# lixilinx/psgd_tf

Measured on AMD Instinct MI355X. Metric: uvd_update_apply_params_per_sec, higher is better.
Workload: dtype f32

## Files before the change

### psgd_tf_amd/csrc/psgd_kron.hip

```cpp
#include <hip/hip_runtime.h>
#include <stdint.h>
#include <stdlib.h>
#include <algorithm>
#include <map>
#include <mutex>
#include <utility>
#include "psgd_hip.h"
#include "kron_shared.h"
#include "nanmax.h"
using psgd::amaxf;
using psgd::nmaxf;

namespace psgdk {

typedef float f32x4 __attribute__((ext_vector_type(4)));

constexpr int kThreads = 256;

enum { EPI_STORE = 0, EPI_TRIU_MAX = 1, EPI_D_MINUS = 2 };

struct GemmArgs {
  const float* A; long a_rs, a_cs;
  const float* B; long b_rs, b_cs;
  const float* A2; long a2_rs, a2_cs;
// ... 1626 lines not shown
    SmallSrc sa, sb;
    small_src_init(sa, ta, m0, hi);
    small_src_init(sb, tb, n0, hi);
    float ra[D][8], rb[D][8];
#pragma unroll
    for (int d = 0; d < D; ++d) {
      small_fetch(sa, lo + d * GK, d < n, ra[d]);
      small_fetch(sb, lo + d * GK, d < n, rb[d]);
    }
    for (int t0 = 0; t0 < n; t0 += D) {
#pragma unroll
      for (int d = 0; d < D; ++d) {
        const int t = t0 + d, buf = d & 1;
        if (t < n) {
          small_commit(sa, lo + t * GK, mul, ra[d], LA + buf * kBuf);
          small_commit(sb, lo + t * GK, 1.0f, rb[d], LB + buf * kBuf);
        }
        small_fetch(sa, lo + (t + D) * GK, t + D < n, ra[d]);
        small_fetch(sb, lo + (t + D) * GK, t + D < n, rb[d]);
        if (t < n) {
          __syncthreads();
#pragma unroll
          for (int kk = 0; kk < GK / 4; ++kk) {
            const int kr = kk * 4 + (lane >> 4);
            const float a = L.A[buf][kr][wm * 16 + (lane & 15)];
            const float b = L.B[buf][kr][wn * 16 + (lane & 15)];
            acc[0][0] = __builtin_amdgcn_mfma_f32_16x16x4f32(a, b, acc[0][0], 0, 0, 0);
          }
        }
      }
    }
    __syncthreads();
  };
  if (nk[0] > 0) run_pair(TileSrc{g.A, g.a_rs, g.a_cs, g.M}, TileSrc{g.B, g.b_cs, g.b_rs, g.N}, klo[0], khi[0], nk[0], a_mul);
  if (nk[1] > 0) run_pair(TileSrc{g.A2, g.a2_rs, g.a2_cs, g.M}, TileSrc{g.B2, g.b2_cs, g.b2_rs, g.N}, klo[1], khi[1], nk[1], -a_mul);
  gemm_epilogue<32>(g, acc, m0, n0);
}

__global__ __launch_bounds__(kThreads) void k_gemm_small(GemmBatch b) {
  __shared__ __attribute__((aligned(16))) GemmLds<32, kSmallK> L;
  int p = 0;
  while (p + 1 < b.count && (int)blockIdx.x >= b.tile_end[p]) ++p;
  const int t = blockIdx.x - (p ? b.tile_end[p - 1] : 0);
  const GemmArgs& g = b.g[p];
  const int tn = (g.N + 31) / 32;
  gemm_body_small(g, (t / tn) * 32, (t % tn) * 32, L);
}

__global__ __launch_bounds__(kThreads) void k_gemm_small_one(GemmArgs g) {
  __shared__ __attribute__((aligned(16))) GemmLds<32, kSmallK> L;
  gemm_body_small(g, blockIdx.y * 32, blockIdx.x * 32, L);
}

constexpr int kMaxGrams = 16;
struct GramBatch {
  int count;
  int tile_end[kMaxGrams];
  const float* Q[kMaxGrams];
  float* P[kMaxGrams];
  int n[kMaxGrams];
};

__host__ __device__ inline GemmArgs gram_args(const float* Q, float* P, int n) {
  GemmArgs g = {};
  g.A = Q; g.a_rs = 1; g.a_cs = n;
  g.B = Q; g.b_rs = n; g.b_cs = 1;
  g.C = P; g.ldc = n; g.M = n; g.N = n; g.K = n;
  g.epi = EPI_STORE;
  g.kmode = KHI_M | KHI_N;
  g.sym = 1;
  return g;
}

template <int T>
__global__ __launch_bounds__(kThreads) void k_gram_batched(GramBatch b) {
  int p = 0;
  while (p + 1 < b.count && (int)blockIdx.x >= b.tile_end[p]) ++p;
  const int t = blockIdx.x - (p ? b.tile_end[p - 1] : 0);
  const GemmArgs g = gram_args(b.Q[p], b.P[p], b.n[p]);
  const int tn = (g.N + T - 1) / T;
  if constexpr (T == 32) {
    __shared__ __attribute__((aligned(16))) GemmLds<32, kSmallK> L;
    gemm_body_small(g, (t / tn) * 32, (t % tn) * 32, L);
  } else {
    __shared__ __attribute__((aligned(16))) GemmLds<T, kSmallK> L;
    gemm_body<T, kSmallK>(g, (t / tn) * T, (t % tn) * T, L);
  }
}

struct TrsmArgs {
  const float* Q; int n, ldq;
  const float* X; float* Y;
  int nvec; long si, sj;
  long xi, xj;
};

__device__ __forceinline__ void trsm_body(const float* __restrict__ Q, int n, int ldq, const float* X, float* Y,
                                          int nvec, long si, long sj, long xi, long xj, int v0,
                                          float (*red)[64][33], float (*Qd)[32]) {
  if (xi == 0 && xj == 0) { xi = si; xj = sj; }
  const int lane = threadIdx.x & 63, w = threadIdx.x >> 6;
  for (int j0 = 0; j0 < n; j0 += 32) {
    const int jw = (n - j0 < 32) ? (n - j0) : 32;
    f32x4 acc[4][2];
#pragma unroll
    for (int i = 0; i < 4; ++i)
// ... 434 lines not shown
  __shared__ float Ybuf[2][512];
  trsm_reg_full_body(t, Dinv, blockIdx.x * 16, Ybuf);
}

__global__ __launch_bounds__(kThreads) void k_tri_inv512(const float* __restrict__ Q, int n, const float* __restrict__ dinv,
                                                         float* __restrict__ Inv, float* amax) {
  __shared__ float Ybuf[2][512];
  const int d = blockIdx.x >> 5, v0 = (blockIdx.x & 31) * 16;
  const long o = (long)(512 * d) * n + 512 * d;
  TrsmArgs t = {Q + o, 512, n, nullptr, Inv + o, 512, (long)n, 1L, 0L, 0L};
  trsm_reg_full_body<true>(t, dinv + (long)(16 * d) * 1024, v0, Ybuf, amax);
}

__global__ __launch_bounds__(kThreads) void k_trsm_ut_reg(TrsmArgs t, const float* __restrict__ Dinv) {
  __shared__ float Ybuf[2][512];
  trsm_reg_body(t, Dinv, blockIdx.x * 16, Ybuf);
}

struct TrsmBatch {
  int count;
  int blk_end[kMaxBatch];
  TrsmArgs t[kMaxBatch];
  const float* dinv[kMaxBatch];
};

__global__ __launch_bounds__(kThreads) void k_trsm_ut_inv_batched(TrsmBatch b, int pitch_max) {
  extern __shared__ __attribute__((aligned(16))) float dyn_lds[];
  int p = 0;
  while (p + 1 < b.count && (int)blockIdx.x >= b.blk_end[p]) ++p;
  const int blk = blockIdx.x - (p ? b.blk_end[p - 1] : 0);
  const TrsmArgs& t = b.t[p];
  const int pitch = ((t.n + 31) & ~31) + 2;
  trsm_inv_body<16>(t, b.dinv[p], blk * 16, dyn_lds, pitch, reinterpret_cast<float (*)[33]>(dyn_lds + 16 * pitch_max));
}

__global__ __launch_bounds__(kThreads) void k_trsm_ut_reg_batched(TrsmBatch b) {
  __shared__ float Ybuf[2][512];
  int p = 0;
  while (p + 1 < b.count && (int)blockIdx.x >= b.blk_end[p]) ++p;
  const int blk = blockIdx.x - (p ? b.blk_end[p - 1] : 0);
  trsm_reg_body(b.t[p], b.dinv[p], blk * 16, Ybuf);
}


struct MixBatch {
  int count, strips;
  int blk_end[kMaxLayers];
  int tile_end[kMaxLayers];
  TrsmArgs t[kMaxLayers];
  const float* dinv[kMaxLayers];
  GemmArgs g[kMaxLayers];
};

__global__ __launch_bounds__(kThreads) void k_small_stage_mixed(MixBatch b) {
  __shared__ __attribute__((aligned(16))) GemmLds<32, kSmallK> L;
  __shared__ float Ybuf[2][512];
  if ((int)blockIdx.x < b.strips) {
    int p = 0;
    while (p + 1 < b.count && (int)blockIdx.x >= b.blk_end[p]) ++p;
    const int blk = blockIdx.x - (p ? b.blk_end[p - 1] : 0);
    trsm_reg_body(b.t[p], b.dinv[p], blk * 16, Ybuf);
    return;
  }
  const int id = blockIdx.x - b.strips;
  int p = 0;
  while (p + 1 < b.count && id >= b.tile_end[p]) ++p;
  const int t = id - (p ? b.tile_end[p - 1] : 0);
  const GemmArgs& g = b.g[p];
  const int tn = (g.N + 31) / 32;
  gemm_body_small(g, (t / tn) * 32, (t % tn) * 32, L);
}

struct BalanceBatch {
  int count;
  const float* Ql[kMaxBatch]; const float* Qr[kMaxBatch];
  float* QlS[kMaxBatch]; float* QrS[kMaxBatch];
  float* dinv[kMaxBatch];
  float* scal[kMaxBatch];
  int M[kMaxBatch], N[kMaxBatch];
};

__device__ __forceinline__ float balance_rho(const float* __restrict__ Ql, const float* __restrict__ Qr, int M, int N,
                                             float (*red)[4]) {
  float ml = -INFINITY, mr = -INFINITY;
  for (int i0 = threadIdx.x; i0 < M; i0 += 8 * kThreads) {
    float x[8];
#pragma unroll
    for (int u = 0; u < 8; ++u) { const long i = min(i0 + u * kThreads, M - 1); x[u] = Ql[i * M + i]; }
#pragma unroll
    for (int u = 0; u < 8; ++u) ml = nmaxf(ml, x[u]);
  }
  for (int i0 = threadIdx.x; i0 < N; i0 += 8 * kThreads) {
    float x[8];
#pragma unroll
    for (int u = 0; u < 8; ++u) { const long i = min(i0 + u * kThreads, N - 1); x[u] = Qr[i * N + i]; }
#pragma unroll
    for (int u = 0; u < 8; ++u) mr = nmaxf(mr, x[u]);
  }
#pragma unroll
  for (int off = 32; off > 0; off >>= 1) {
    ml = nmaxf(ml, __shfl_down(ml, off, 64));
    mr = nmaxf(mr, __shfl_down(mr, off, 64));
  }
  const int lane = threadIdx.x & 63, w = threadIdx.x >> 6;
  if (lane == 0) { red[0][w] = ml; red[1][w] = mr; }
  __syncthreads();
  ml = nmaxf(nmaxf(red[0][0], red[0][1]), nmaxf(red[0][2], red[0][3]));
  mr = nmaxf(nmaxf(red[1][0], red[1][1]), nmaxf(red[1][2], red[1][3]));
  return sqrtf(ml / mr);
}

__device__ __forceinline__ void balance_body(const float* __restrict__ Ql, const float* __restrict__ Qr, int M, int N,
                                             float* QlS, float* QrS, float (*red)[4], int bid, int nblocks,
                                             float* part_l = nullptr, float* part_r = nullptr) {
  const float rho = balance_rho(Ql, Qr, M, N, red);
  const long nl = (long)M * M, nr = (long)N * N;
  const long tid = (long)bid * kThreads + threadIdx.x, nth = (long)nblocks * kThreads;
  float ml = 0.0f, mr = 0.0f;
  const bool v4 = ((reinterpret_cast<uintptr_t>(Ql) | reinterpret_cast<uintptr_t>(Qr) | reinterpret_cast<uintptr_t>(QlS) |
                    reinterpret_cast<uintptr_t>(QrS)) & 15) == 0;
  long dl = 0, dr = 0;
  if (v4) {
    const long nl4 = nl >> 2, nr4 = nr >> 2;
// ... 548 lines not shown
  return (lo >= kInvMinSmall && hi >= kInvMinN) || (lo >= 512 && hi >= 2560) || (lo >= 256 && hi >= 4096);
}

static KronWs kron_layout(char* base, int M, int N) {
  KronWs k;
  const int64_t mm = (int64_t)M * M * 4, nn = (int64_t)N * N * 4, mn = (int64_t)M * N * 4;
  int64_t off = 0;
  auto take = [&](int64_t bytes) { float* p = reinterpret_cast<float*>(base + off); off = align256(off + bytes); return p; };
  k.scal = take(256);
  k.QlS = take(mm); k.QrS = take(nn);
  k.T = take(mn); k.A = take(mn); k.X1 = take(mn); k.Bt = take(mn);
  k.g1 = take(mm); k.g2 = take(nn);
  k.dinv = take((int64_t)((M + 31) / 32 + (N + 31) / 32) * 1024 * 4);
  k.Pl = take(mm); k.Pr = take(nn);
  k.PP = k.F1 = k.F2 = k.Y0 = k.Y1 = k.Y2 = nullptr;
  k.Lr = k.Lc = k.Rr = k.Rc = k.G1 = k.G2 = k.U0 = k.U1 = k.U2 = k.U3 = nullptr;
  k.split_scratch = nullptr; k.split_cnt = nullptr; k.S0 = nullptr;
  k.sk_scratch = nullptr; k.sk_cnt = nullptr; k.pmeta = nullptr; k.pm_part = nullptr; k.te = nullptr;
  k.IcL = k.IcR = k.TpL = k.TpR = k.DXp = k.X1p = nullptr; k.TfL = k.TfR = nullptr;
  if (kron_planes(M, N)) {
    const int64_t Mp = pad128(M), Np = pad128(N), small = Mp < Np ? Mp : Np, big = Mp < Np ? Np : Mp;
    auto planes = [&](int64_t elems) { return reinterpret_cast<__bf16*>(take(elems * 6)); };
    k.PP = planes(small * small); k.F1 = planes(big * big); k.F2 = planes(big * big);
    k.Y0 = planes(Mp * Np); k.Y1 = planes(Mp * Np); k.Y2 = planes(Mp * Np);
    k.Lr = planes(Mp * Mp); k.Lc = planes(Mp * Mp); k.G1 = planes(Mp * Mp);
    k.Rr = planes(Np * Np); k.Rc = planes(Np * Np); k.G2 = planes(Np * Np);
    k.U0 = planes(Mp * Np); k.U1 = planes(Mp * Np); k.U2 = planes(Mp * Np); k.U3 = planes(Mp * Np);
    {
      const int64_t T1 = small / 128, nsp = T1 * (T1 + 1) / 2 < kGradSplitMax ? T1 * (T1 + 1) / 2 : kGradSplitMax;
      k.split_scratch = take(nsp * kGradChunks * 64 * kThreads * 4);
      k.split_cnt = reinterpret_cast<unsigned*>(take(2 * kGradSplitMax * 4));
    }
    k.S0 = planes(big * 2048);
    k.pmeta = reinterpret_cast<PlaneMeta*>(take(1024));
    k.pm_part = take(4 * 2048 * 4);
    k.te = reinterpret_cast<int*>(take((int64_t)kTeSlots * kTeLd * kTeLd * 4));
    if (kron_inv_route(M, N)) {
      k.IcL = planes(Mp * Mp); k.TpL = planes(Mp * Mp); k.TfL = take(mm);
      k.IcR = planes(Np * Np); k.TpR = planes(Np * Np); k.TfR = take(nn);
      k.DXp = planes(Mp * Np); k.X1p = planes(Mp * Np);
    }
    if (kron_t128(M, N) <= kSkMaxTiles) {
      k.sk_scratch = take((int64_t)kSkItems * 64 * kThreads * 4);
      k.sk_cnt = reinterpret_cast<unsigned*>(take(kSkMaxTiles * 4));
    }
  }
  k.total = off;
  return k;
}

static int g_gemm_x3 = 1;
static int g_force_gemm = 0;
static int g_small_deep = 1;

static int x3_host_mode(const float* P, long rs, long cs) {
  if (rs == 1 && cs > 0 && cs < (1L << 23)) return X3_XROW;
  if (cs == 1 && rs > 0 && rs < (1L << 22) && (rs & 3) == 0 && (reinterpret_cast<uintptr_t>(P) & 15) == 0) return X3_KVEC;
  return X3_EDGE;
}
static void x3_host_modes(const GemmArgs& g, int& ma, int& mb) {
  ma = x3_host_mode(g.A, g.a_rs, g.a_cs);
  mb = x3_host_mode(g.B, g.b_cs, g.b_rs);
  if (g.A2 && (x3_host_mode(g.A2, g.a2_rs, g.a2_cs) != ma || x3_host_mode(g.B2, g.b2_cs, g.b2_rs) != mb)) ma = X3_EDGE;
  if (ma == X3_EDGE || mb == X3_EDGE) ma = mb = X3_EDGE;
}

template <bool LITE>
static void launch_x3(const GemmArgs& g, dim3 grid, hipStream_t st) {
  int ma, mb;
  x3_host_modes(g, ma, mb);
  if (ma == X3_KVEC && mb == X3_XROW) hipLaunchKernelGGL((k_gemm_x3<X3_KVEC, X3_XROW, LITE>), grid, dim3(kThreads), 0, st, g);
  else if (ma == X3_KVEC && mb == X3_KVEC) hipLaunchKernelGGL((k_gemm_x3<X3_KVEC, X3_KVEC, LITE>), grid, dim3(kThreads), 0, st, g);
  else if (ma == X3_XROW && mb == X3_XROW) hipLaunchKernelGGL((k_gemm_x3<X3_XROW, X3_XROW, LITE>), grid, dim3(kThreads), 0, st, g);
  else if (ma == X3_XROW && mb == X3_KVEC) hipLaunchKernelGGL((k_gemm_x3<X3_XROW, X3_KVEC, LITE>), grid, dim3(kThreads), 0, st, g);
  else hipLaunchKernelGGL((k_gemm_x3<X3_EDGE, X3_EDGE, LITE>), grid, dim3(kThreads), 0, st, g);
}

static int launch_gemm(const GemmArgs& g, hipStream_t st) {
  if (g.C == g.A || g.C == g.B || (g.A2 && (g.C == g.A2 || g.C == g.B2))) return PSGD_ERR_BAD_ARG;
  const long t128 = (long)((g.N + 127) / 128) * ((g.M + 127) / 128);
  const long t64 = (long)((g.N + 63) / 64) * ((g.M + 63) / 64);
  int T = t128 >= 64 ? 128 : (t64 >= 48 ? 64 : 32);
  if (g_force_gemm == 1) T = 64;
  if (g_force_gemm == 2) T = 128;
  if (g_force_gemm == 3) T = 32;
  dim3 grid((g.N + T - 1) / T, (g.M + T - 1) / T);
  if (T == 128 && g_gemm_x3 && g.lite) launch_x3<true>(g, grid, st);
  else if (T == 128 && g_gemm_x3) launch_x3<false>(g, grid, st);
  else if (T == 128) hipLaunchKernelGGL((k_gemm_f32<128, kBigK>), grid, dim3(kThreads), 0, st, g);
  else if (T == 64) hipLaunchKernelGGL((k_gemm_f32<64, kSmallK>), grid, dim3(kThreads), 0, st, g);
  else if (g_small_deep && g.K > 2 * kSmallK)
    hipLaunchKernelGGL(k_gemm_small_one, grid, dim3(kThreads), 0, st, g);
  else hipLaunchKernelGGL((k_gemm_f32<32, kSmallK>), grid, dim3(kThreads), 0, st, g);
  return (int)hipGetLastError();
}

static bool gemm_uses_x3(const GemmArgs& g) {
  const long t128 = (long)((g.N + 127) / 128) * ((g.M + 127) / 128);
  return g_gemm_x3 && (g_force_gemm == 0 ? t128 >= 64 : g_force_gemm == 2);
}

static int launch_gemm_two(const GemmArgs& a, const GemmArgs& b, hipStream_t st) {
  if (!gemm_uses_x3(a) || !gemm_uses_x3(b)) {
    const int rc = launch_gemm(a, st);
    return rc ? rc : launch_gemm(b, st);
  }
  GemmPair p;
  p.g[0] = a; p.g[1] = b;
  p.tx0 = (a.N + 127) / 128; p.tx1 = (b.N + 127) / 128;
  p.tiles0 = p.tx0 * ((a.M + 127) / 128);
  const int tiles1 = p.tx1 * ((b.M + 127) / 128);
  p.tiles1 = tiles1;
  int ma0, mb0, ma1, mb1;
  x3_host_modes(a, ma0, mb0);
  x3_host_modes(b, ma1, mb1);
  const dim3 grid(p.tiles0 + tiles1);
  if (ma0 == X3_KVEC && mb0 == X3_KVEC && ma1 == X3_XROW && mb1 == X3_XROW)
    hipLaunchKernelGGL((k_gemm_x3_pair<X3_KVEC, X3_KVEC, X3_XROW, X3_XROW>), grid, dim3(kThreads), 0, st, p);
  else if (ma0 == X3_KVEC && mb0 == X3_XROW && ma1 == X3_KVEC && mb1 == X3_XROW)
    hipLaunchKernelGGL((k_gemm_x3_pair<X3_KVEC, X3_XROW, X3_KVEC, X3_XROW>), grid, dim3(kThreads), 0, st, p);
  else {
    const int rc = launch_gemm(a, st);
    return rc ? rc : launch_gemm(b, st);
  }
  return (int)hipGetLastError();
}

static GemmArgs gemm_args(const float* A, int lda, bool ta, const float* B, int ldb, bool tb, float* C, int ldc, int M,
                          int N, int K, int kmode = 0) {
  GemmArgs g = {};
  g.A = A; g.a_rs = ta ? 1 : lda; g.a_cs = ta ? lda : 1;
  g.B = B; g.b_rs = tb ? 1 : ldb; g.b_cs = tb ? ldb : 1;
  g.C = C; g.ldc = ldc; g.M = M; g.N = N; g.K = K;
  g.epi = EPI_STORE;
  g.kmode = kmode;
  return g;
}

constexpr int kSmallKron = 512;
static inline bool kron_small(int M, int N) { return M <= kSmallKron && N <= kSmallKron; }

static void plan_apply(const float* Ql, const float* Qr, const float* G, float* out, int M, int N, const KronWs& k,
                       GemmArgs (&pre)[2], int& np, GemmArgs (&app)[3], int& na) {
// ... 318 lines not shown
        (long)((cw + 127) / 128) * ((nvec + 127) / 128) >= g_trsm_planes_min_tiles && (!Qc->meta || strip_slots > 0)) {
      P3Buf Yg = {blk, pad128(nvec), kw};
      int e;
      if (Qc->meta) {
        Yg.meta = strip_meta++; --strip_slots;
        if ((e = launch_absmax_view(Y + (long)k0 * sj, si, sj, nvec, kw, Yg, part, st))) return e;
      }
      if ((e = launch_split3(Y + (long)k0 * sj, si, sj, nvec, kw, Yg, st))) return e;
      P3Args g = p3_args(Yg, *Qc, nvec, cw, kw, 0);
      g.B.p = Qc->p + (long)(k0 / 32) * (Qc->rows * 32) + (long)c0 * 32;
      float* Yr = Y + (long)c0 * sj;
      g.e.C = Yr; g.e.ldc = si; g.e.c_cs = sj;
      g.e.D = (lazy && k0 == 0 ? X : Y) + (long)c0 * sj; g.e.ldd = si;
      g.e.epi = EPI_D_MINUS;
      return launch_p3(g, st);
    }
    GemmArgs g = {};
    g.A = Y + (long)k0 * sj; g.a_rs = si; g.a_cs = sj;
    g.B = Q + (long)k0 * n + c0; g.b_rs = n; g.b_cs = 1;
    float* Yr = Y + (long)c0 * sj;
    g.C = Yr; g.ldc = si; g.c_cs = sj;
    g.D = (lazy && k0 == 0 ? X : Y) + (long)c0 * sj; g.ldd = si;
    g.M = nvec; g.N = cw; g.K = kw;
    g.epi = EPI_D_MINUS;
    g.lite = lite;
    return launch_gemm(g, st);
  };
  const int group = kTrsmBlock * (g_trsm_group > 0 ? g_trsm_group : (n >= 8 * kTrsmBlock ? 4 : 1));
  for (int g0 = 0; g0 < n; g0 += group) {
    const int gend = (n - g0 < group) ? n : g0 + group;
    for (int j0 = g0; j0 < gend; j0 += kTrsmBlock) {
      const int jw = (gend - j0 < kTrsmBlock) ? (gend - j0) : kTrsmBlock;
      float* Yb = Y + (long)j0 * sj;
      TrsmArgs t = {Q + (long)j0 * n + j0, jw, n, (lazy && j0 == 0) ? X : Yb, Yb, nvec, si, sj, 0L, 0L};
      int e = launch_strip(t, dinv + (long)(j0 / 32) * 1024, st);
      if (e) return e;
      if (j0 + jw < gend && (e = update(j0, jw, j0 + jw, gend - j0 - jw))) return e;
    }
    if (gend < n) {
      const int e = update(g0, gend - g0, gend, n - gend);
      if (e) return e;
    }
  }
  return 0;
}

static int launch_gemm_batch(const GemmArgs* g, int count, hipStream_t st) {
  GemmBatch b;
  b.count = count;
  long t64 = 0;
  for (int p = 0; p < count; ++p) t64 += (long)((g[p].N + 63) / 64) * ((g[p].M + 63) / 64);
  const int T = t64 >= 96 ? 64 : 32;
  int tiles = 0;
  for (int p = 0; p < count; ++p) {
    b.g[p] = g[p];
    tiles += ((g[p].N + T - 1) / T) * ((g[p].M + T - 1) / T);
    b.tile_end[p] = tiles;
  }
  if (T == 64) hipLaunchKernelGGL((k_gemm_f32_batched<64>), dim3(tiles), dim3(kThreads), 0, st, b);
  else if (g_small_deep) hipLaunchKernelGGL(k_gemm_small, dim3(tiles), dim3(kThreads), 0, st, b);
  else hipLaunchKernelGGL((k_gemm_f32_batched<32>), dim3(tiles), dim3(kThreads), 0, st, b);
  return (int)hipGetLastError();
}

static int launch_gram_batch(const GemmArgs* g, int count, hipStream_t st) {
  for (int p0 = 0; p0 < count; p0 += kMaxGrams) {
    GramBatch b;
    b.count = (count - p0 < kMaxGrams) ? count - p0 : kMaxGrams;
    long t64 = 0;
    for (int p = 0; p < b.count; ++p) t64 += (long)((g[p0 + p].N + 63) / 64) * ((g[p0 + p].M + 63) / 64);
    const int T = t64 >= 96 ? 64 : 32;
    int tiles = 0;
    for (int p = 0; p < b.count; ++p) {
      const GemmArgs& a = g[p0 + p];
      b.Q[p] = a.A; b.P[p] = a.C; b.n[p] = a.M;
      tiles += ((a.N + T - 1) / T) * ((a.M + T - 1) / T);
      b.tile_end[p] = tiles;
    }
    if (T == 64) hipLaunchKernelGGL((k_gram_batched<64>), dim3(tiles), dim3(kThreads), 0, st, b);
    else hipLaunchKernelGGL((k_gram_batched<32>), dim3(tiles), dim3(kThreads), 0, st, b);
    if (hipGetLastError() != hipSuccess) return 1;
  }
  return 0;
}

static int launch_p3_two(const P3Args& a, const P3Args& b, hipStream_t st) {
  P3Pair p;
  p.g[0] = a; p.g[1] = b;
  p.tx0 = (a.e.N + 127) / 128; p.tx1 = (b.e.N + 127) / 128;
  p.tiles0 = p.tx0 * ((a.e.M + 127) / 128);
  const int tiles1 = p.tx1 * ((b.e.M + 127) / 128);
  p.tiles1 = tiles1;
  const dim3 grid(p.tiles0 + tiles1);
  const bool none = p3_no_early((p.tiles0 + tiles1) / 2 >= p3_block_slots() * 3 / 4);
  if (!a.fmt) hipLaunchKernelGGL((k_gemm_p3_pair<0, 2>), grid, dim3(kThreads), 0, st, p);
  else if (p3_uses_te(a) || p3_uses_te(b)) {
    if (none) hipLaunchKernelGGL((k_gemm_p3_pair<1, 0, true>), grid, dim3(kThreads), 0, st, p);
    else hipLaunchKernelGGL((k_gemm_p3_pair<1, 2, true>), grid, dim3(kThreads), 0, st, p);
  } else if (none) hipLaunchKernelGGL((k_gemm_p3_pair<1, 0>), grid, dim3(kThreads), 0, st, p);
  else hipLaunchKernelGGL((k_gemm_p3_pair<1, 2>), grid, dim3(kThreads), 0, st, p);
  return (int)hipGetLastError();
}

static int g_grad_rect = 1;
static int g_grad_split = 1;
constexpr int g_grad_order = 1;
static int grad_rect_chunks(int m_long, int k_long, int k_short) {
  if (!g_grad_split || !g_grad_rect || k_long == k_short) return 0;
  const int Tl = (m_long + 127) / 128, nl = Tl * (Tl + 1) / 2;
  const int ratio = (k_long + k_short / 2) / k_short;
  if (ratio < 2 || nl > kGradSplitMax) return 0;
  const int nchunk = ratio >= 7 ? 8 : ratio >= 5 ? 6 : ratio >= 3 ? 4 : 2;
// ... 715 lines not shown
  if (!f || !f->bg || hipStreamWaitEvent(f->bg, f->fork, 0) != hipSuccess) return 1;
  f->bg_live = 1;
  return 0;
}

int kron_join(KronFork* f, hipStream_t main) {
  if (f->bg_live) {
    f->bg_live = 0;
    if (hipEventRecord(f->bg_done, f->bg) != hipSuccess || hipStreamWaitEvent(main, f->bg_done, 0) != hipSuccess) return 1;
  }
  if (hipEventRecord(f->join, f->side) != hipSuccess) return 1;
  return hipStreamWaitEvent(main, f->join, 0) != hipSuccess;
}

}

using namespace psgdk;

#define KRON_LAUNCH(expr)                     \
  do {                                        \
    if ((expr) != 0) return PSGD_ERR_LAUNCH;  \
  } while (0)

static int kron_ws_check(void* ws, int64_t ws_bytes, int64_t need) {
  if (!ws || (reinterpret_cast<uintptr_t>(ws) & 255) || ws_bytes < need) return PSGD_ERR_WORKSPACE;
  return PSGD_OK;
}

extern "C" {

int psgd_kron_set_tuning(int key, int value) {
  if (key == 0) { g_force_gemm = value; return PSGD_OK; }
  if (key == 1) { g_gemm_x3 = value; return PSGD_OK; }
  if (key == 2) { g_trsm_lds = value; return PSGD_OK; }
  if (key == 3) { g_small_deep = value; return PSGD_OK; }
  if (key == 4) { g_planes = value; return PSGD_OK; }
  if (key == 6) { g_grad_split = value; return PSGD_OK; }
  if (key == 7) { g_stage_mix = value; return PSGD_OK; }
  if (key == 9) { g_overlap = value; return PSGD_OK; }
  if (key == 11) { g_trsm_inv = value; return PSGD_OK; }
  if (key == 12) { g_planes_f16 = value; return PSGD_OK; }
  if (key == 16) { g_planes_exact = value; return PSGD_OK; }
  if (key == 23) { g_inv_strip512 = value; return PSGD_OK; }
  if (key == 24) { g_inv_blk = value; return PSGD_OK; }
  if (key == 25) { g_inv_order = value; return PSGD_OK; }
  if (key == 27) { g_pair_order = value; return PSGD_OK; }
  if (key == 28) { g_tile_scales = value; return PSGD_OK; }
  if (key == 29) { g_x0_side = value; return PSGD_OK; }
  if (key == 30) { g_bg_front = value; return PSGD_OK; }
  if (key == 31) { g_fused_prologue = value; return PSGD_OK; }
  if (key == 32) { g_bg_planes = value; return PSGD_OK; }
  if (key == 33) { g_grad_rect = value; return PSGD_OK; }
  if (key == 34) { g_solve_split = value; return PSGD_OK; }
  return PSGD_ERR_BAD_ARG;
}

int64_t psgd_kron_dd_workspace_bytes(int M, int N) {
  if (M <= 0 || N <= 0) return PSGD_ERR_BAD_ARG;
  return kron_layout(nullptr, M, N).total;
}

static inline bool kron_apply_planes(int M, int N) { return kron_planes_apply(M, N) && g_planes && g_gemm_x3; }

int psgd_kron_dd_prepare_f32(const float* Ql, const float* Qr, int M, int N, void* ws, int64_t ws_bytes, void* stream) {
  if (!Ql || !Qr) return PSGD_ERR_BAD_ARG;
  if (M <= 0 || N <= 0) return PSGD_ERR_SHAPE;
  if (kron_ws_check(ws, ws_bytes, kron_layout(nullptr, M, N).total)) return PSGD_ERR_WORKSPACE;
  hipStream_t st = static_cast<hipStream_t>(stream);
  KronWs k = kron_layout(static_cast<char*>(ws), M, N);
  if (kron_apply_planes(M, N)) {
    KRON_LAUNCH(planes_prepare(Ql, Qr, M, N, k, st));
    return PSGD_OK;
  }
  GemmArgs pre[2], app[3];
  int np = 0, na = 0;
  plan_apply(Ql, Qr, Ql , k.T , M, N, k, pre, np, app, na);
  if (np == 2) KRON_LAUNCH(launch_gram_batch(pre, 2, st));
  else KRON_LAUNCH(launch_gemm(pre[0], st));
  return PSGD_OK;
}

int psgd_kron_dd_apply_prepared_f32(const float* Ql, const float* Qr, const float* G, float* out, int M, int N, void* ws,
                                    int64_t ws_bytes, void* stream) {
  if (!Ql || !Qr || !G || !out) return PSGD_ERR_BAD_ARG;
  if (M <= 0 || N <= 0) return PSGD_ERR_SHAPE;
  if (kron_ws_check(ws, ws_bytes, kron_layout(nullptr, M, N).total)) return PSGD_ERR_WORKSPACE;
  hipStream_t st = static_cast<hipStream_t>(stream);
  KronWs k = kron_layout(static_cast<char*>(ws), M, N);
  if (kron_apply_planes(M, N)) {
    KRON_LAUNCH(planes_apply(G, out, M, N, k, st));
    return PSGD_OK;
  }
  GemmArgs pre[2], app[3];
  int np = 0, na = 0;
  plan_apply(Ql, Qr, G, out, M, N, k, pre, np, app, na);
  for (int i = 0; i < na; ++i) KRON_LAUNCH(launch_gemm(app[i], st));
  return PSGD_OK;
}

int psgd_kron_dd_apply_f32(const float* Ql, const float* Qr, const float* G, float* out, int M, int N, void* ws,
                           int64_t ws_bytes, void* stream) {
  const int rc = psgd_kron_dd_prepare_f32(Ql, Qr, M, N, ws, ws_bytes, stream);
  if (rc) return rc;
  return psgd_kron_dd_apply_prepared_f32(Ql, Qr, G, out, M, N, ws, ws_bytes, stream);
}

// ... 246 lines not shown
                                    const float* const* dG, float* const* QlOut, float* const* QrOut, const int* M,
                                    const int* N, int count, float step, float tiny, void* ws, int64_t ws_bytes,
                                    void* stream) {
  if (!Ql || !Qr || !dX || !dG || !QlOut || !QrOut || !M || !N || count <= 0) return PSGD_ERR_BAD_ARG;
  const int64_t need = psgd_kron_dd_workspace_bytes_batched(M, N, count);
  if (need < 0) return (int)need;
  if (kron_ws_check(ws, ws_bytes, need)) return PSGD_ERR_WORKSPACE;
  for (int p = 0; p < count; ++p)
    if (M[p] > 512 || N[p] > 512) return PSGD_ERR_SHAPE;
  hipStream_t st = static_cast<hipStream_t>(stream);
  char* base = static_cast<char*>(ws);
  for (int p0 = 0; p0 < count; p0 += kMaxLayers) {
    const int nb = (count - p0 < kMaxLayers) ? count - p0 : kMaxLayers;
    GemmArgs s[kMaxLayers][6];
    KronWs k[kMaxLayers];
    BalanceBatch bb;
    TrsmBatch t1, t2;
    bb.count = t1.count = t2.count = nb;
    int blk1 = 0, blk2 = 0, nmax = 0;
    for (int q = 0; q < nb; ++q) {
      const int p = p0 + q;
      if (!Ql[p] || !Qr[p] || !dX[p] || !dG[p] || !QlOut[p] || !QrOut[p]) return PSGD_ERR_BAD_ARG;
      k[q] = kron_layout(base, M[p], N[p]);
      base += k[q].total;
      plan_update(dG[p], QlOut[p], QrOut[p], M[p], N[p], step, tiny, k[q], s[q]);
      bb.Ql[q] = Ql[p]; bb.Qr[q] = Qr[p]; bb.QlS[q] = k[q].QlS; bb.QrS[q] = k[q].QrS; bb.M[q] = M[p]; bb.N[q] = N[p];
      bb.scal[q] = k[q].scal; bb.dinv[q] = k[q].dinv;
      t1.t[q] = {k[q].QrS, N[p], N[p], dX[p], k[q].X1, M[p], (long)N[p], 1L, 0L, 0L};
      t1.dinv[q] = k[q].dinv; t2.dinv[q] = k[q].dinv + (long)((N[p] + 31) / 32) * 1024;
      t2.t[q] = {k[q].QlS, M[p], M[p], k[q].X1, k[q].Bt, N[p], 1L, (long)N[p], 0L, 0L};
      blk1 += (M[p] + 15) / 16; t1.blk_end[q] = blk1;
      blk2 += (N[p] + 15) / 16; t2.blk_end[q] = blk2;
      if (M[p] > nmax) nmax = M[p];
      if (N[p] > nmax) nmax = N[p];
    }
    hipLaunchKernelGGL(k_kron_balance_batched, dim3(kBalInvBlocks + 64, nb), dim3(kThreads), 0, st, bb);
    KRON_LAUNCH((int)hipGetLastError());
    GemmArgs g[kMaxBatch];
    long t64 = 0;
    for (int q = 0; q < nb; ++q) t64 += (long)((N[p0 + q] + 63) / 64) * ((M[p0 + q] + 63) / 64);
    const bool mixed = (g_stage_mix & 1) && t64 < 96 && g_small_deep && !g_trsm_lds;
    if (mixed) {
      for (int stage = 0; stage < 2; ++stage) {
        MixBatch mb;
        const TrsmBatch& tb = stage ? t2 : t1;
        mb.count = nb; mb.strips = stage ? blk2 : blk1;
        int tiles = 0;
        for (int q = 0; q < nb; ++q) {
          mb.blk_end[q] = tb.blk_end[q]; mb.t[q] = tb.t[q]; mb.dinv[q] = tb.dinv[q];
          mb.g[q] = s[q][stage];
          tiles += ((mb.g[q].N + 31) / 32) * ((mb.g[q].M + 31) / 32);
          mb.tile_end[q] = tiles;
        }
        hipLaunchKernelGGL(k_small_stage_mixed, dim3(mb.strips + tiles), dim3(kThreads), 0, st, mb);
        KRON_LAUNCH((int)hipGetLastError());
      }
    }
    for (int stage = 0; stage < 2 && !mixed; ++stage) {
      for (int q = 0; q < nb; ++q) g[q] = s[q][stage];
      KRON_LAUNCH(launch_gemm_batch(g, nb, st));
    }
    for (int pass = 0; pass < 2 && !mixed; ++pass) {
      TrsmBatch& tb = pass ? t2 : t1;
      if (!g_trsm_lds) {
        hipLaunchKernelGGL(k_trsm_ut_reg_batched, dim3(pass ? blk2 : blk1), dim3(kThreads), 0, st, tb);
        KRON_LAUNCH((int)hipGetLastError());
        continue;
      }
      const int pitch_max = ((nmax + 31) & ~31) + 2;
      static DeviceOnce attr_set;
      if (attr_set.needed()) {
        if (hipFuncSetAttribute(reinterpret_cast<const void*>(&k_trsm_ut_inv_batched),
                                hipFuncAttributeMaxDynamicSharedMemorySize,
                                (int)((64 * (kStripN + 2) + 32 * 33) * sizeof(float))) != hipSuccess)
          return PSGD_ERR_LAUNCH;
        attr_set.done();
      }
      hipLaunchKernelGGL(k_trsm_ut_inv_batched, dim3(pass ? blk2 : blk1), dim3(kThreads),
                         (size_t)(16 * pitch_max + 32 * 33) * sizeof(float), st, tb, pitch_max);
      KRON_LAUNCH((int)hipGetLastError());
    }
    for (int stage = 2; stage < 6; stage += 2) {
      for (int q = 0; q < nb; ++q) { g[2 * q] = s[q][stage]; g[2 * q + 1] = s[q][stage + 1]; }
      KRON_LAUNCH(launch_gemm_batch(g, 2 * nb, st));
    }
  }
  return PSGD_OK;
}


struct SparseWs {
  float *scal, *LS, *RS, *T, *A, *Bt, *gsq, *v0, *v1, *v2, *v3, *dinv, *cpart;
  __bf16 *P0, *P1;
  float* sk_scratch; unsigned* sk_cnt;
  __bf16* GP[2][2]; PlaneMeta* gmeta; float* gpart; int64_t gcap;
  __bf16 *IQc, *IIr, *IIc, *ITp; float *IInv, *ITf; PlaneMeta* imeta;
  int64_t total;
};

constexpr int kSplitkMaxTiles = 160, kSplitkScratchTiles = 640;
static inline bool sparse_splitk(int rows, int K) {
  const long T = (rows + 127) / 128;
  return T * (T + 1) / 2 <= kSplitkMaxTiles && K >= 4096;
}

static SparseWs sparse_layout(char* base, int fmt, int M, int N) {
  SparseWs k;
// ... 386 lines not shown
```

Baseline: 9.699 billion.

## Add split-K small GEMM kernel with wave-level K partitioning and LDS reduction

Adds a 32x32-tile GEMM path for small non-symmetric problems. Each of the four wavefronts takes a slice of the K range, loads operands straight from global memory into registers with a D-deep prefetch, runs MFMA 16x16x4 f32, and the partial sums are combined through LDS. It is used by the single, batched and mixed-stage small GEMM launches under a new toggle that defaults on. The aim is to cut per-tile latency on deep-K small tiles by running waves in parallel along K instead of staging through LDS. The cost is uncoalesced strided global loads and an extra LDS reduction.

```diff
diff --git a/psgd_tf_amd/csrc/psgd_kron.hip b/psgd_tf_amd/csrc/psgd_kron.hip
--- a/psgd_tf_amd/csrc/psgd_kron.hip
+++ b/psgd_tf_amd/csrc/psgd_kron.hip
@@ -1702,6 +1702,126 @@
   gemm_body_small(g, blockIdx.y * 32, blockIdx.x * 32, L);
 }
 
+constexpr int kSplitD = 8;
+
+template <int D>
+__device__ __forceinline__ void gemm_body_splitk(const GemmArgs& g, int m0, int n0, float* R) {
+  const int lane = threadIdx.x & 63, w = __builtin_amdgcn_readfirstlane(threadIdx.x >> 6);
+  const int r16 = lane & 15, h = lane >> 4;
+  const bool tri_skip = (g.epi == EPI_TRIU_MAX || g.sym) && (m0 >= n0 + 32);
+  if (g.sym && tri_skip) return;
+
+  f32x4 acc[2][2];
+#pragma unroll
+  for (int i = 0; i < 2; ++i)
+#pragma unroll
+    for (int j = 0; j < 2; ++j) acc[i][j] = f32x4{0.f, 0.f, 0.f, 0.f};
+
+  auto run_pair = [&](const TileSrc& ta, const TileSrc& tb, int lo, int hi, float sign) {
+    const int ns = (hi - lo + 3) >> 2;
+    const int q = (ns + 3) >> 2;
+    const int s_lo = w * q;
+    const int n = min(ns, s_lo + q) - s_lo;
+    unsigned offa[2], offb[2];
+#pragma unroll
+    for (int i = 0; i < 2; ++i) {
+      offa[i] = (unsigned)((long)min(m0 + 16 * i + r16, ta.X - 1) * ta.rs + (long)(lo + h) * ta.cs);
+      offb[i] = (unsigned)((long)min(n0 + 16 * i + r16, tb.X - 1) * tb.rs + (long)(lo + h) * tb.cs);
+    }
+    const unsigned sa = 4u * (unsigned)ta.cs, sb = 4u * (unsigned)tb.cs;
+    auto fetch = [&](int s, float (&a)[2], float (&b)[2]) {
+      const int sg = s_lo + s;
+      const bool ok = (s < n) && (lo + 4 * sg + h < hi);
+#pragma unroll
+      for (int i = 0; i < 2; ++i) {
+        a[i] = ta.P[ok ? offa[i] + (unsigned)sg * sa : 0u];
+        b[i] = tb.P[ok ? offb[i] + (unsigned)sg * sb : 0u];
+      }
+    };
+    float ra[D][2], rb[D][2];
+#pragma unroll
+    for (int d = 0; d < D; ++d) fetch(d, ra[d], rb[d]);
+    float mul = sign;
+    if (g.scale_max) mul = sign * (g.step / (g.scale_max[0] + g.tiny));
+    for (int s0 = 0; s0 < n; s0 += D) {
+#pragma unroll
+      for (int d = 0; d < D; ++d) {
+        const int s = s0 + d;
+        if (s < n) {
+          const bool ok = lo + 4 * (s_lo + s) + h < hi;
+          float a[2], b[2];
+#pragma unroll
+          for (int i = 0; i < 2; ++i) {
+            a[i] = ok ? ra[d][i] * mul : 0.0f;
+            b[i] = ok ? rb[d][i] : 0.0f;
+          }
+#pragma unroll
+          for (int i = 0; i < 2; ++i)
+#pragma unroll
+            for (int j = 0; j < 2; ++j) acc[i][j] = __builtin_amdgcn_mfma_f32_16x16x4f32(a[i], b[j], acc[i][j], 0, 0, 0);
+        }
+        fetch(s + D, ra[d], rb[d]);
+      }
+    }
+  };
+
+  f32x4 out[1][1] = {{f32x4{0.f, 0.f, 0.f, 0.f}}};
+  if (!tri_skip) {
+    for (int p = 0; p < (g.A2 ? 2 : 1); ++p) {
+      const int K = p ? g.K2 : g.K, km = p ? g.kmode2 : g.kmode;
+      int lo = 0, hi = K;
+      if (km & KLO_M) lo = max(lo, m0);
+      if (km & KLO_N) lo = max(lo, n0);
+      if (km & KHI_M) hi = min(hi, m0 + 32);
+      if (km & KHI_N) hi = min(hi, n0 + 32);
+      if (hi <= lo) continue;
+      if (p == 0) run_pair(TileSrc{g.A, g.a_rs, g.a_cs, g.M}, TileSrc{g.B, g.b_cs, g.b_rs, g.N}, lo, hi, 1.0f);
+      else run_pair(TileSrc{g.A2, g.a2_rs, g.a2_cs, g.M}, TileSrc{g.B2, g.b2_cs, g.b2_rs, g.N}, lo, hi, -1.0f);
+    }
+#pragma unroll
+    for (int i = 0; i < 2; ++i)
+#pragma unroll
+      for (int j = 0; j < 2; ++j)
+#pragma unroll
+        for (int e = 0; e < 4; ++e) R[(w * 16 + (i * 2 + j) * 4 + e) * 64 + lane] = acc[i][j][e];
+    __syncthreads();
+#pragma unroll
+    for (int e = 0; e < 4; ++e) {
+      float v = R[(0 * 16 + w * 4 + e) * 64 + lane];
+#pragma unroll
+      for (int p = 1; p < 4; ++p) v += R[(p * 16 + w * 4 + e) * 64 + lane];
+      out[0][0][e] = v;
+    }
+  }
+  gemm_epilogue<32>(g, out, m0, n0);
+}
+
+constexpr int kSplitLds = 4 * 16 * 64;
+
+template <int NMAX>
+__device__ __forceinline__ int batch_problem(const int (&tile_end)[NMAX], int count, int id) {
+  int p = 0;
+#pragma unroll
+  for (int q = 0; q + 1 < NMAX; ++q) p += (q + 1 < count && id >= tile_end[q]) ? 1 : 0;
+  return p;
+}
+
+template <int D>
+__global__ __launch_bounds__(kThreads) void k_gemm_small_split(GemmBatch b) {
+  __shared__ __attribute__((aligned(16))) float R[kSplitLds];
+  const int p = batch_problem(b.tile_end, b.count, (int)blockIdx.x);
+  const int t = blockIdx.x - (p ? b.tile_end[p - 1] : 0);
+  const GemmArgs& g = b.g[p];
+  const int tn = (g.N + 31) / 32;
+  gemm_body_splitk<D>(g, (t / tn) * 32, (t % tn) * 32, R);
+}
+
+template <int D>
+__global__ __launch_bounds__(kThreads) void k_gemm_small_split_one(GemmArgs g) {
+  __shared__ __attribute__((aligned(16))) float R[kSplitLds];
+  gemm_body_splitk<D>(g, blockIdx.y * 32, blockIdx.x * 32, R);
+}
+
 constexpr int kMaxGrams = 16;
 struct GramBatch {
   int count;
@@ -2242,8 +2362,8 @@
   GemmArgs g[kMaxLayers];
 };
 
+template <bool SPLIT>
 __global__ __launch_bounds__(kThreads) void k_small_stage_mixed(MixBatch b) {
-  __shared__ __attribute__((aligned(16))) GemmLds<32, kSmallK> L;
   __shared__ float Ybuf[2][512];
   if ((int)blockIdx.x < b.strips) {
     int p = 0;
@@ -2253,12 +2373,22 @@
     return;
   }
   const int id = blockIdx.x - b.strips;
-  int p = 0;
-  while (p + 1 < b.count && id >= b.tile_end[p]) ++p;
-  const int t = id - (p ? b.tile_end[p - 1] : 0);
-  const GemmArgs& g = b.g[p];
-  const int tn = (g.N + 31) / 32;
-  gemm_body_small(g, (t / tn) * 32, (t % tn) * 32, L);
+  if constexpr (SPLIT) {
+    __shared__ __attribute__((aligned(16))) float R[kSplitLds];
+    const int p = batch_problem(b.tile_end, b.count, id);
+    const int t = id - (p ? b.tile_end[p - 1] : 0);
+    const GemmArgs& g = b.g[p];
+    const int tn = (g.N + 31) / 32;
+    gemm_body_splitk<kSplitD>(g, (t / tn) * 32, (t % tn) * 32, R);
+  } else {
+    __shared__ __attribute__((aligned(16))) GemmLds<32, kSmallK> L;
+    int p = 0;
+    while (p + 1 < b.count && id >= b.tile_end[p]) ++p;
+    const int t = id - (p ? b.tile_end[p - 1] : 0);
+    const GemmArgs& g = b.g[p];
+    const int tn = (g.N + 31) / 32;
+    gemm_body_small(g, (t / tn) * 32, (t % tn) * 32, L);
+  }
 }
 
 struct BalanceBatch {
@@ -2913,6 +3043,7 @@
 static int g_gemm_x3 = 1;
 static int g_force_gemm = 0;
 static int g_small_deep = 1;
+static int g_small_split = 1;
 
 static int x3_host_mode(const float* P, long rs, long cs) {
   if (rs == 1 && cs > 0 && cs < (1L << 23)) return X3_XROW;
@@ -2950,6 +3081,8 @@
   else if (T == 128 && g_gemm_x3) launch_x3<false>(g, grid, st);
   else if (T == 128) hipLaunchKernelGGL((k_gemm_f32<128, kBigK>), grid, dim3(kThreads), 0, st, g);
   else if (T == 64) hipLaunchKernelGGL((k_gemm_f32<64, kSmallK>), grid, dim3(kThreads), 0, st, g);
+  else if (g_small_split && !g.sym && g_small_deep) hipLaunchKernelGGL(k_gemm_small_split_one<kSplitD>, grid, dim3(kThreads), 0, st, g);
+  else if (g_small_split && !g.sym) hipLaunchKernelGGL(k_gemm_small_split_one<1>, grid, dim3(kThreads), 0, st, g);
   else if (g_small_deep && g.K > 2 * kSmallK)
     hipLaunchKernelGGL(k_gemm_small_one, grid, dim3(kThreads), 0, st, g);
   else hipLaunchKernelGGL((k_gemm_f32<32, kSmallK>), grid, dim3(kThreads), 0, st, g);
@@ -3374,12 +3507,16 @@
   for (int p = 0; p < count; ++p) t64 += (long)((g[p].N + 63) / 64) * ((g[p].M + 63) / 64);
   const int T = t64 >= 96 ? 64 : 32;
   int tiles = 0;
+  bool split = g_small_split != 0;
   for (int p = 0; p < count; ++p) {
     b.g[p] = g[p];
     tiles += ((g[p].N + T - 1) / T) * ((g[p].M + T - 1) / T);
     b.tile_end[p] = tiles;
+    if (g[p].sym) split = false;
   }
   if (T == 64) hipLaunchKernelGGL((k_gemm_f32_batched<64>), dim3(tiles), dim3(kThreads), 0, st, b);
+  else if (split && g_small_deep) hipLaunchKernelGGL(k_gemm_small_split<kSplitD>, dim3(tiles), dim3(kThreads), 0, st, b);
+  else if (split) hipLaunchKernelGGL(k_gemm_small_split<1>, dim3(tiles), dim3(kThreads), 0, st, b);
   else if (g_small_deep) hipLaunchKernelGGL(k_gemm_small, dim3(tiles), dim3(kThreads), 0, st, b);
   else hipLaunchKernelGGL((k_gemm_f32_batched<32>), dim3(tiles), dim3(kThreads), 0, st, b);
   return (int)hipGetLastError();
@@ -4201,6 +4338,7 @@
   if (key == 32) { g_bg_planes = value; return PSGD_OK; }
   if (key == 33) { g_grad_rect = value; return PSGD_OK; }
   if (key == 34) { g_solve_split = value; return PSGD_OK; }
+  if (key == 35) { g_small_split = value; return PSGD_OK; }
   return PSGD_ERR_BAD_ARG;
 }
 
@@ -4553,7 +4691,8 @@
           tiles += ((mb.g[q].N + 31) / 32) * ((mb.g[q].M + 31) / 32);
           mb.tile_end[q] = tiles;
         }
-        hipLaunchKernelGGL(k_small_stage_mixed, dim3(mb.strips + tiles), dim3(kThreads), 0, st, mb);
+        if (g_small_split) hipLaunchKernelGGL(k_small_stage_mixed<true>, dim3(mb.strips + tiles), dim3(kThreads), 0, st, mb);
+        else hipLaunchKernelGGL(k_small_stage_mixed<false>, dim3(mb.strips + tiles), dim3(kThreads), 0, st, mb);
         KRON_LAUNCH((int)hipGetLastError());
       }
     }
```

After: 9.675 billion. Within noise of the previous version (-0.2%).
